# zju3dv/LoFTR

Measured on AMD Instinct MI355X. Metric: image-pairs/sec @640x480 indoor-ds, higher is better.
Workload: dtype f32; 1 GPU; batch=8 640x480 synthetic grayscale pairs per GPU, indoor_ds dual-softmax (BASELINE configs[1]), full LoFTR.forward = ResNet-FPN backbone (HIP implicit-GEMM / patch convolutions incl. the 7x7 stem) + HIP matching path; weights=seeded random init (no checkpoint on the box), conf_matrix_materialised=True, match_type=dual_softmax, global_batch=8, parallelism=dp1 (pairs sharded; RCCL all-gather of match counts)

## Files before the change

include/loftr_hip.h:

```cpp
#ifndef LOFTR_HIP_H_
#define LOFTR_HIP_H_

#include <stddef.h>
#include <stdint.h>

#ifdef __cplusplus
extern "C" {
#endif

typedef enum {
  LOFTR_OK = 0,
  LOFTR_ERR_BAD_ARG = -1,
  LOFTR_ERR_UNSUPPORTED = -2,
  LOFTR_ERR_WORKSPACE = -3,
  LOFTR_ERR_LAUNCH = -4,
  LOFTR_ERR_NO_DEVICE = -5,
  LOFTR_ERR_COMM = -6,
  LOFTR_ERR_RANGE = -7
} loftr_status;

#define LOFTR_HIP_ABI_VERSION 25

int loftr_hip_abi_version(void);
const char* loftr_hip_status_string(int status);
// ... 126 lines not shown
                                 const float* merge_b, float* out0, float* out1, void* ws,
                                 size_t ws_bytes, void* stream);

int loftr_window_head(const uint32_t* h_sp0, const uint32_t* h_sp1, int N, int H, int Wm, int Cin,
                      const void* prepared, size_t prepared_bytes, int Cout, const int64_t* b_ids,
                      const int64_t* i_ids, const int64_t* j_ids, int M, int w0c, int w1c, int stride, int W,
                      uint32_t* win0_sp, uint32_t* win1_sp, void* stream);
int loftr_fine_preprocess_window_head(const uint32_t* h_sp0, const uint32_t* h_sp1, int N, int H, int Wm, int Cin,
                                      const void* prepared, size_t prepared_bytes,
                                      const float* feat_c0, const float* feat_c1, int L, int S, int Cc,
                                      const int64_t* b_ids, const int64_t* i_ids, const int64_t* j_ids, int M,
                                      int w0c, int w1c, int stride, int W, int Cf,
                                      const float* down_w, const float* down_b, const float* merge_w,
                                      const float* merge_b, float* out0, float* out1, void* ws, size_t ws_bytes,
                                      void* stream);

int loftr_fine_match(const float* feat_f0, const float* feat_f1, int M, int WW, int C,
                     const float* mkpts1_c, const int64_t* b_ids, float scale,
                     const float* scale1, float* expec_f, float* mkpts1_f, void* stream);

size_t loftr_conv_workspace_bytes(int Cin, int Cout, int KH, int KW);
int loftr_conv_bn_act(const uint32_t* x_sp, int B, int H, int W, int Cin, const float* weight,
                      const long* weight_strides, int Cout, int KH, int KW, int stride, int pad, const float* bn_weight, const float* bn_bias,
                      const float* bn_mean, const float* bn_var, float bn_eps, int act,
                      const uint32_t* residual_sp, uint32_t* y_sp, float* y_f32, void* ws, size_t ws_bytes,
                      const float* x_inv_scale, void* stream);
int loftr_conv_prepare(const float* weight, const long* weight_strides, int Cin, int Cout, int KH, int KW,
                       const float* bn_weight, const float* bn_bias, const float* bn_mean, const float* bn_var,
                       float bn_eps, void* prepared, size_t prepared_bytes, void* stream);
#define LOFTR_CONV_SHARED_GPU 0x100
// ... 122 lines not shown
```

loftr_amd/_lib.py:

```python
import ctypes as C
import os

HERE = os.path.dirname(os.path.abspath(__file__))
LIB_PATH = os.environ.get("LOFTR_HIP_LIB") or os.path.join(HERE, "libloftr_hip.so")

_p = C.c_void_p
_i = C.c_int
_f = C.c_float
_sz = C.c_size_t
_l = C.c_long


class LayerWeights(C.Structure):
    _fields_ = [(n, _p) for n in ("q_proj", "k_proj", "v_proj", "merge", "mlp0", "mlp2",
                                  "norm1_w", "norm1_b", "norm2_w", "norm2_b")]


class CoarseParams(C.Structure):
    _fields_ = [("N", _i), ("h0c", _i), ("w0c", _i), ("h1c", _i), ("w1c", _i), ("C", _i),
                ("thr", _f), ("border_rm", _i), ("scale", _f),
                ("mask0", _p), ("mask1", _p), ("scale0", _p), ("scale1", _p)]


class MatchOut(C.Structure):
# ... 36 lines not shown
    "loftr_coarse_match_sinkhorn": (_i, [_p, _p, C.POINTER(CoarseParams), _f, _i, _i, _p, _p, C.POINTER(MatchOut),
                                         _p, _sz, _p]),
    "loftr_fine_preprocess_workspace_bytes": (_sz, [_i, _i, _i]),
    "loftr_fine_preprocess": (_i, [C.POINTER(FMap), C.POINTER(FMap), _p, _p, _i, _i, _i, _p, _p, _p, _i, _i, _i, _i,
                                   _i, _i, _p, _p, _p, _p, _p, _p, _p, _sz, _p]),
    "loftr_fine_preprocess_bwd_workspace_bytes": (_sz, [_i, _i, _i, _i]),
    "loftr_fine_preprocess_bwd": (_i, [C.POINTER(FMap), C.POINTER(FMap), _p, _p, _i, _i, _i, _p, _p, _p, _i, _i, _i, _i, _i, _i,
                                       _p, _p, _p, _p, _p, C.POINTER(FMap), C.POINTER(FMap), _p, _p, _p, _p, _p, _p, _p, _sz, _p]),
    "loftr_fine_match": (_i, [_p, _p, _i, _i, _i, _p, _p, _f, _p, _p, _p, _p]),
    "loftr_pos_encode_flatten_gather": (_i, [C.POINTER(FMap), _i, _p, _i, _p, _i, _i, _p, _i, _p]),
    "loftr_fine_preprocess_gather": (_i, [C.POINTER(FMap), _i, _p, C.POINTER(FMap), _i, _p, _p, _p, _i, _i, _i, _p, _p, _p, _i, _i, _i, _i,
                                          _i, _i, _p, _p, _p, _p, _p, _p, _p, _sz, _p]),
    "loftr_window_head": (_i, [_p, _p, _i, _i, _i, _i, _p, _sz, _i, _p, _p, _p, _i, _i, _i, _i, _i, _p, _p, _p]),
    "loftr_fine_preprocess_window_head": (_i, [_p, _p, _i, _i, _i, _i, _p, _sz, _p, _p, _i, _i, _i, _p, _p, _p, _i, _i, _i, _i,
                                               _i, _i, _p, _p, _p, _p, _p, _p, _p, _sz, _p]),
    "loftr_conv_workspace_bytes": (_sz, [_i, _i, _i, _i]),
    "loftr_conv_bn_act": (_i, [_p, _i, _i, _i, _i, _p, C.POINTER(_l), _i, _i, _i, _i, _i, _p, _p, _p, _p, _f, _i, _p, _p, _p, _p, _sz, _p, _p]),
    "loftr_stem_conv_bn_relu": (_i, [_p, C.POINTER(_l), _i, _i, _i, _p, C.POINTER(_l), _i, _p, _p, _p, _p, _f, _p, _p]),
    "loftr_upsample2x_add": (_i, [_p, _p, _p, _i, _i, _i, _i, _p]),
    "loftr_bn_train_workspace_bytes": (_sz, [_i, _i, _l]),
    "loftr_bn_train_fwd": (_i, [_p, _i, _i, _l, _i, _p, _p, _f, _p, _p, _p, _p, _p, _sz, _p]),
    "loftr_bn_train_bwd": (_i, [_p, _p, _i, _i, _l, _i, _p, _p, _p, _p, _p, _p, _p, _sz, _p]),
    "loftr_act_fwd": (_i, [_p, _p, _l, _i, _f, _p, _p]),
    "loftr_act_bwd": (_i, [_p, _p, _l, _i, _f, _p, _p]),
    "loftr_upsample2x_bilinear_fwd": (_i, [_p, _i, _i, _i, _i, _i, _p, _p]),
    "loftr_upsample2x_bilinear_bwd": (_i, [_p, _i, _i, _i, _i, _i, _p, _p]),
    "loftr_resize_linear_u8": (_i, [_p, _i, _i, _l, _p, _i, _i, _l, _p]),
    "loftr_pack_gray_u8": (_i, [_p, _l, _l, _p, _i, _i, _i, _p, _p, _p, _i, _p]),
    "loftr_epipolar_errors": (_i, [_p, _p, _p, _p, _p, _p, _l, _i, _p, _p]),
    "loftr_spvs_coarse_workspace_bytes": (_sz, [_i, _i, _i]),
# ... 79 lines not shown
```

loftr_amd/backbone.py:

```python
import os

import torch
import torch.nn as nn
import torch.nn.functional as F

from . import autograd, ops

FUSE_TOPDOWN = os.environ.get("LOFTR_FUSE_TOPDOWN", "1") != "0"


TRAIN_CONV_HIP = os.environ.get("LOFTR_TRAIN_CONV", "1") != "0"


class Conv2d(nn.Conv2d):

    def forward(self, x):
        if (TRAIN_CONV_HIP and self.training and x.is_cuda and x.dtype == torch.float32 and torch.is_grad_enabled()
                and self.in_channels <= 256 and (x.requires_grad or self.weight.requires_grad)):
            return autograd.conv2d(x, self.weight, self.stride[0], self.padding[0])
        return super().forward(x)


TRAIN_GLUE_HIP = os.environ.get("LOFTR_TRAIN_GLUE", "1") != "0"
GLUE_PARTS = set(os.environ.get("LOFTR_TRAIN_GLUE_PARTS", "bn,act,add,up").split(","))
# ... 165 lines not shown
        self.layer1_outconv2 = _fuse_head(d2, d1)
        self._init()

    def forward(self, x):
        x0 = self.relu(self.bn1(self.conv1(x)))
        x1 = self.layer1(x0)
        x2 = self.layer2(x1)
        x3 = self.layer3(x2)
        x3_out = self.layer3_outconv(x3)
        x2_out = self.layer2_outconv2(self.layer2_outconv(x2) + self._up(x3_out))
        x1_out = self.layer1_outconv2(self.layer1_outconv(x1) + self._up(x2_out))
        return [x3_out, x1_out]

    WINDOW_HEAD = "layer1_outconv2"

    def fine_head_last(self, h_sp):
        head = self.layer1_outconv2
        _, x1_f32 = ops.conv_bn_act(h_sp, head[0].out_channels, head[3], None, act=0, want_sp=False, want_f32=True)
        return self._nchw_view(x1_f32)

    @torch.no_grad()
    def forward_hip(self, x, defer_fine=False, head_input=False):
        assert defer_fine or not head_input
        a0 = self._stem_hip(x)
        a1 = self._stage_hip(self.layer1, a0)
        a2 = self._stage_hip(self.layer2, a1)
        a3 = self._stage_hip(self.layer3, a2)
        d3 = self.layer3_outconv.out_channels
        x3_sp, x3_f32 = ops.conv_bn_act(a3[0], a3[1], self.layer3_outconv, want_f32=True)

        def fine():
            t2 = self._topdown_hip(a2, self.layer2_outconv, x3_sp, d3)
            x2_out, _ = self._head_hip(self.layer2_outconv2, (t2, d3), want_f32=False, shared_gpu=defer_fine)
            d2 = self.layer2_outconv2[3].out_channels
            t1 = self._topdown_hip(a1, self.layer1_outconv, x2_out, d2)
            if head_input:
                head = self.layer1_outconv2
                return ops.conv_bn_act(t1, d2, head[0], head[1], act=2, shared_gpu=defer_fine)[0]
            _, x1_f32 = self._head_hip(self.layer1_outconv2, (t1, d2), want_f32=True, shared_gpu=defer_fine)
            return self._nchw_view(x1_f32)

        if defer_fine:
            fine.reads = (a1[0], a2[0], x3_sp)
            return [self._nchw_view(x3_f32), fine]
        return [self._nchw_view(x3_f32), fine()]


class ResNetFPN_16_4(_ResNetFPN):
    _HIP_STAGES = ("layer1", "layer2", "layer3", "layer4")
    _HIP_OUTCONVS = ("layer4_outconv", "layer3_outconv", "layer2_outconv")
# ... 64 lines not shown
```

loftr_amd/build.py:

```python
import os
import subprocess
import sys
from concurrent.futures import ThreadPoolExecutor

HERE = os.path.dirname(os.path.abspath(__file__))
CSRC = os.path.join(HERE, "csrc")
OBJ_DIR = os.path.join(CSRC, "build")
LIB_PATH = os.path.join(HERE, "libloftr_hip.so")
SOURCES = ["linear.hip", "coarse_plan.hip", "attention.hip", "transformer.hip", "coarse_match.hip", "fine.hip", "misc.hip",
           "sp_convert.hip", "conv.hip", "eval.hip", "input.hip", "comm.hip", "pose.hip", "train.hip", "train_bwd.hip", "encoder_fused.hip", "fine_fused.hip", "head_grads.hip", "encoder_bwd.hip", "fine_bwd.hip", "train_glue.hip", "bank.hip", "pose_gpu.hip", "window_head.hip", "geometry.hip", "geometry_gpu.hip"]
FLAGS = ["--offload-arch=gfx950", "-O3", "-std=c++17", "-fPIC", "-Wall", "-Wno-unused-parameter"]


def _hipcc():
    for c in (os.environ.get("HIPCC"), "/opt/rocm/bin/hipcc", "hipcc"):
        if c and (os.path.isabs(c) and os.path.exists(c) or not os.path.isabs(c)):
            return c
    raise RuntimeError("hipcc not found")


def _deps_mtime():
    paths = [os.path.join(CSRC, f) for f in os.listdir(CSRC) if f.endswith((".h", ".hip"))]
    paths.append(os.path.join(os.path.dirname(HERE), "include", "loftr_hip.h"))
    return max(os.path.getmtime(p) for p in paths)

# ... 51 lines not shown
```

loftr_amd/loftr.py:

```python
import contextlib
import math
import warnings
import weakref

import torch
import torch.nn as nn

from . import autograd, ops
from .backbone import build_backbone


class PositionEncodingSine(nn.Module):

    def __init__(self, d_model, max_shape=(256, 256), temp_bug_fix=True):
        super().__init__()
        ys = torch.arange(1, max_shape[0] + 1, dtype=torch.float32).view(1, -1, 1).expand(1, *max_shape)
        xs = torch.arange(1, max_shape[1] + 1, dtype=torch.float32).view(1, 1, -1).expand(1, *max_shape)
        idx = torch.arange(0, d_model // 2, 2).float()
        if temp_bug_fix:
            freq = torch.exp(idx * (-math.log(10000.0) / (d_model // 2)))
        else:
            freq = torch.exp(idx * (-math.log(10000.0) / d_model // 2))
        freq = freq[:, None, None]
        pe = torch.zeros((d_model, *max_shape))
# ... 214 lines not shown
        return {"b_ids": b_ids, "i_ids": i_ids, "j_ids": j_ids, "gt_mask": ~predicted, "m_bids": b_ids[predicted],
                "mkpts0_c": pts0[predicted], "mkpts1_c": pts1[predicted], "mconf": mconf[predicted]}


class FinePreprocess(nn.Module):

    def __init__(self, config):
        super().__init__()
        self.config = config
        self.cat_c_feat = config["fine_concat_coarse_feat"]
        self.W = self.config["fine_window_size"]
        d_model_c = self.config["coarse"]["d_model"]
        d_model_f = self.config["fine"]["d_model"]
        self.d_model_f = d_model_f
        self.last_head = None
        if self.cat_c_feat:
            self.down_proj = nn.Linear(d_model_c, d_model_f, bias=True)
            self.merge_feat = nn.Linear(2 * d_model_f, d_model_f, bias=True)
        for p in self.parameters():
            if p.dim() > 1:
                nn.init.kaiming_normal_(p, mode="fan_out", nonlinearity="relu")

    def forward(self, feat_f0, feat_f1, feat_c0, feat_c1, data):
        W = self.W
        stride = data["hw0_f"][0] // data["hw0_c"][0]
        data.update({"W": W})
        if data["b_ids"].shape[0] == 0:
            feat0 = torch.empty(0, self.W ** 2, self.d_model_f, device=feat_f0.device)
            feat1 = torch.empty(0, self.W ** 2, self.d_model_f, device=feat_f0.device)
            return feat0, feat1
# ... 16 lines not shown
        dense_pixels = 2 * h_sp0.shape[0] * h_sp0.shape[1] * h_sp0.shape[2]
        windows = fine_head == "windows" or ops.window_head_wins(M, dense_pixels)
        if M == 0 or not windows or not ops.window_head_supported(self.W, cin, conv.out_channels, h_sp0, h_sp1):
            self.last_head = "dense"
            if M == 0:
                return self.forward(h_sp0, h_sp1, feat_c0, feat_c1, data)
            return self.forward(dense_fn(h_sp0), dense_fn(h_sp1), feat_c0, feat_c1, data)
        self.last_head = "windows"
        W = self.W
        stride = data["hw0_f"][0] // data["hw0_c"][0]
        data.update({"W": W})
        return ops.fine_preprocess_windows(h_sp0, h_sp1, cin, conv, feat_c0, feat_c1, data["b_ids"], data["i_ids"], data["j_ids"],
                                           tuple(data["hw0_c"]), tuple(data["hw1_c"]), W, stride,
                                           down_w=self.down_proj.weight, down_b=self.down_proj.bias,
                                           merge_w=self.merge_feat.weight, merge_b=self.merge_feat.bias)

    def forward_gather(self, bank_f0, slot0, bank_f1, slot1, feat_c0, feat_c1, data):
        W = self.W
        stride = data["hw0_f"][0] // data["hw0_c"][0]
        data.update({"W": W})
        if data["b_ids"].shape[0] == 0:
            feat0 = torch.empty(0, self.W ** 2, self.d_model_f, device=bank_f0.device)
            feat1 = torch.empty(0, self.W ** 2, self.d_model_f, device=bank_f0.device)
            return feat0, feat1
        kw = {}
        if self.cat_c_feat:
            kw = dict(down_w=self.down_proj.weight, down_b=self.down_proj.bias,
                      merge_w=self.merge_feat.weight, merge_b=self.merge_feat.bias)
        return ops.fine_preprocess_gather(bank_f0, slot0, bank_f1, slot1, feat_c0, feat_c1, data["b_ids"], data["i_ids"], data["j_ids"],
                                          tuple(data["hw0_c"]), tuple(data["hw1_c"]), W, stride, **kw)
# ... 52 lines not shown
                or img0.shape[2:] != img1.shape[2:] or not hasattr(self.backbone, "WINDOW_HEAD") or not self.fine_preprocess.cat_c_feat):
            return False
        return img0.shape[0] + img1.shape[0] <= self._backbone_cap(img0)

    def _backbone_cap(self, x):
        return getattr(self, "_backbone_chunk_images", None) or max(1, (2 ** 31 - 1) // ((x.shape[2] // 2) * (x.shape[3] // 2) * 256))

    def run_backbone(self, data, head_input=False):
        data.update({"bs": data["image0"].size(0),
                     "hw0_i": data["image0"].shape[2:], "hw1_i": data["image1"].shape[2:]})
        cl = lambda img: img.contiguous(memory_format=torch.channels_last)
        use_hip = self.backbone_impl == "hip" and data["image0"].is_cuda and not self.training
        run = self.backbone.forward_hip if use_hip else self.backbone
        self._fine_join = None
        assert not head_input or (use_hip and data["hw0_i"] == data["hw1_i"])
        hkw = dict(head_input=True) if head_input else {}
        if data["hw0_i"] == data["hw1_i"]:
            x = cl(torch.cat([data["image0"], data["image1"]], dim=0))
            cap = self._backbone_cap(x)
            if use_hip and x.shape[0] > cap:
                outs = [run(x[i:i + cap]) for i in range(0, x.shape[0], cap)]
                feats_c, feats_f = torch.cat([o[0] for o in outs]), torch.cat([o[1] for o in outs])
            elif use_hip and self.overlap_fine_branch and (data["bs"] >= 8 if self.backbone_halves is None else self.backbone_halves):
                main = torch.cuda.current_stream(x.device)
                self.backbone.prepare_hip()
                if self._half_streams is None:
                    self._half_streams = [torch.cuda.Stream(device=x.device) for _ in range(2)]
                outs, fines, evs = [], [], []
                for k, st in enumerate(self._half_streams):
                    st.wait_stream(main)
                    xk = data["image0"] if k == 0 else data["image1"]
# ... 39 lines not shown
            self._fine_join = None

    def match_from_features(self, feat_c0, feat_c1, feat_f0, feat_f1, data, head_input=False):
        data.update({"hw0_c": feat_c0.shape[2:], "hw1_c": feat_c1.shape[2:]})
        if head_input:
            data.update({"hw0_f": feat_f0.shape[1:3], "hw1_f": feat_f1.shape[1:3]})
        else:
            data.update({"hw0_f": feat_f0.shape[2:], "hw1_f": feat_f1.shape[2:]})
        both = (ops.stacked_halves(feat_c0, feat_c1)
                if feat_c0.shape == feat_c1.shape and not autograd.wants_grad(feat_c0, feat_c1) else None)
        if both is not None:
            feat_c0, feat_c1 = self.pos_encoding(both).split(feat_c0.shape[0])
        else:
            feat_c0 = self.pos_encoding(feat_c0)
            feat_c1 = self.pos_encoding(feat_c1)
        if head_input:
            head = getattr(self.backbone, self.backbone.WINDOW_HEAD)
            fine_pre = lambda c0, c1: self.fine_preprocess.forward_windows(feat_f0, feat_f1, head[0].out_channels, head[3], self.backbone.fine_head_last,
                                                                           self.fine_head, c0, c1, data)
        else:
            fine_pre = lambda c0, c1: self.fine_preprocess(feat_f0, feat_f1, c0, c1, data)
        self._match_encoded(feat_c0, feat_c1, data, fine_pre)

    def _match_encoded(self, feat_c0, feat_c1, data, fine_preprocess):
        mask_c0 = mask_c1 = None
        if "mask0" in data:
            mask_c0, mask_c1 = data["mask0"].flatten(-2), data["mask1"].flatten(-2)
        feat_c0, feat_c1 = self.loftr_coarse(feat_c0, feat_c1, mask_c0, mask_c1, inplace=True, mode=self.coarse_mode,
                                             skip_padded=self.skip_padded_tiles and mask_c0 is not None)
        if not self.fine_join_late:
            self._join_fine(feat_c0.device)
# ... 17 lines not shown
            self.fine_matching(feat_f0_unfold, feat_f1_unfold, data)

    def forward(self, data):
        graph = self.training and self.full_grads and torch.is_grad_enabled()
        with torch.enable_grad() if graph else torch.no_grad():
            return self._forward(data)

    def _forward(self, data):
        dev = data["image0"].device
        if data["image1"].device != dev:
            raise ops._lib.LoftrHipError(f"image0 on {dev} but image1 on {data['image1'].device}")
        if dev.type != "cuda":
            feat_c0, feat_c1, feat_f0, feat_f1 = self.run_backbone(data)
            return self.match_from_features(feat_c0, feat_c1, feat_f0, feat_f1, data)
        with torch.cuda.device(dev):
            head_input = self._window_head_applies(data)
            feat_c0, feat_c1, feat_f0, feat_f1 = self.run_backbone(data, head_input=head_input)
            self.match_from_features(feat_c0, feat_c1, feat_f0, feat_f1, data, head_input=head_input)

    def match_pairs(self, bank0, ids0, bank1=None, ids1=None):
        from .pairs import match_pairs
        return match_pairs(self, bank0, ids0, bank1, ids1)

    def load_state_dict(self, state_dict, *args, **kwargs):
        for k in list(state_dict.keys()):
            if k.startswith("matcher."):
                state_dict[k.replace("matcher.", "", 1)] = state_dict.pop(k)
        return super().load_state_dict(state_dict, *args, **kwargs)
```

loftr_amd/ops.py:

```python
import ctypes as C
import os
import weakref
import functools

import torch

from . import _lib
from ._lib import CoarseParams, FMap, LayerWeights, MatchOut, check

_WS = {}

LAYER_FIELDS = (("q_proj", "q_proj.weight"), ("k_proj", "k_proj.weight"), ("v_proj", "v_proj.weight"),
                ("merge", "merge.weight"), ("mlp0", "mlp.0.weight"), ("mlp2", "mlp.2.weight"),
                ("norm1_w", "norm1.weight"), ("norm1_b", "norm1.bias"),
                ("norm2_w", "norm2.weight"), ("norm2_b", "norm2.bias"))


_PREPARED = weakref.WeakKeyDictionary()


def _tensors_in(obj):
    if isinstance(obj, torch.Tensor):
        yield obj
    elif isinstance(obj, (list, tuple)):
# ... 422 lines not shown
    out = torch.empty(2 * M, W * W, Cf, device=dev, dtype=torch.float32)
    out0, out1 = out[:M], out[M:]
    if M == 0:
        return out0, out1
    lib = _lib.load()
    ws = workspace(lib.loftr_fine_preprocess_workspace_bytes(M, W, Cf), dev)
    N, H, Wm, _ = h_sp0.shape
    check(lib.loftr_fine_preprocess_window_head(_ptr(h_sp0), _ptr(h_sp1), N, H, Wm, Cin, _ptr(prepared), prepared.numel(),
                                                _ptr(feat_c0), _ptr(feat_c1), feat_c0.shape[1], feat_c1.shape[1], feat_c0.shape[2],
                                                *ids, M, hw0_c[1], hw1_c[1], int(stride), int(W), Cf, _ptr(down_w), _ptr(down_b),
                                                _ptr(merge_w), _ptr(merge_b), _ptr(out0), _ptr(out1), _ptr(ws), ws.numel(),
                                                _stream()), "loftr_fine_preprocess_window_head")
    return out0, out1


def _slot_ids(ids, n_slots, name, device):
    host = ids.detach().cpu() if isinstance(ids, torch.Tensor) else torch.as_tensor(ids)
    if host.dim() != 1 or host.dtype.is_floating_point or host.dtype == torch.bool:
        raise _lib.LoftrHipError(f"{name}: expected a 1-D integer tensor of slot ids, got {tuple(host.shape)} {host.dtype}")
    if host.numel() and (int(host.min()) < 0 or int(host.max()) >= n_slots):
        raise _lib.LoftrHipError(f"{name}: slot id out of range [0, {n_slots}) (min {int(host.min())}, max {int(host.max())})")
    if isinstance(ids, torch.Tensor) and ids.is_cuda and ids.dtype == torch.int32 and ids.is_contiguous() and ids.device == device:
        return ids
    return host.to(torch.int32).to(device)


def _bank_map(bank, name):
    if not isinstance(bank, torch.Tensor) or not bank.is_cuda or bank.dtype != torch.float32 or bank.dim() != 4:
        raise _lib.LoftrHipError(f"{name}: expected a 4-D float32 GPU tensor [n_slots, C, H, W]")
    if bank.shape[0] == 0:
# ... 456 lines not shown
```

Before: 408.7 image-pairs/s.

## Compute both fine-head 3x3 convs only on matched windows instead of dense map

Moves the first 3x3 conv+BN+ReLU of layer1_outconv2 out of the dense backbone. It is now computed only over 7x7 neighbourhoods around the matched coarse cells, followed by the second conv on the 5x5 windows. A new MFMA kernel file stages patches and weights through LDS with async global-to-LDS loads. This is meant to skip dense full-resolution conv work when the total window area is small relative to the map. It falls back to the dense path when the fill ratio exceeds a threshold, and it adds a new code path that has to be kept equivalent to the dense one.

New measurement: 434.0 image-pairs/s (median of 6 runs). +6.2%, better.

```diff
diff --git a/include/loftr_hip.h b/include/loftr_hip.h
--- a/include/loftr_hip.h
+++ b/include/loftr_hip.h
@@ -164,6 +164,23 @@
                                       const float* down_w, const float* down_b, const float* merge_w,
                                       const float* merge_b, float* out0, float* out1, void* ws, size_t ws_bytes,
                                       void* stream);
+
+int loftr_window_head_first(const uint32_t* t_sp0, const uint32_t* t_sp1, int N, int H, int Wm, int Cin,
+                            const void* prepared, size_t prepared_bytes, int Cout, const int64_t* b_ids,
+                            const int64_t* i_ids, const int64_t* j_ids, int M, int w0c, int w1c, int stride, int W,
+                            uint32_t* nb_sp, void* stream);
+int loftr_window_head_last(const uint32_t* nb_sp, int H, int Wm, int Cin, const void* prepared, size_t prepared_bytes,
+                           int Cout, const int64_t* b_ids, const int64_t* i_ids, const int64_t* j_ids, int M, int w0c,
+                           int w1c, int stride, int W, uint32_t* win0_sp, uint32_t* win1_sp, void* stream);
+int loftr_fine_preprocess_window_head2(const uint32_t* t_sp0, const uint32_t* t_sp1, int N, int H, int Wm, int Cin,
+                                       const void* prepared0, size_t prepared0_bytes, int Cmid,
+                                       const void* prepared1, size_t prepared1_bytes,
+                                       const float* feat_c0, const float* feat_c1, int L, int S, int Cc,
+                                       const int64_t* b_ids, const int64_t* i_ids, const int64_t* j_ids, int M,
+                                       int w0c, int w1c, int stride, int W, int Cf,
+                                       const float* down_w, const float* down_b, const float* merge_w,
+                                       const float* merge_b, float* out0, float* out1, void* ws, size_t ws_bytes,
+                                       uint32_t* nb_sp, void* stream);
 
 int loftr_fine_match(const float* feat_f0, const float* feat_f1, int M, int WW, int C,
                      const float* mkpts1_c, const int64_t* b_ids, float scale,
diff --git a/loftr_amd/_lib.py b/loftr_amd/_lib.py
--- a/loftr_amd/_lib.py
+++ b/loftr_amd/_lib.py
@@ -74,6 +74,10 @@
     "loftr_window_head": (_i, [_p, _p, _i, _i, _i, _i, _p, _sz, _i, _p, _p, _p, _i, _i, _i, _i, _i, _p, _p, _p]),
     "loftr_fine_preprocess_window_head": (_i, [_p, _p, _i, _i, _i, _i, _p, _sz, _p, _p, _i, _i, _i, _p, _p, _p, _i, _i, _i, _i,
                                                _i, _i, _p, _p, _p, _p, _p, _p, _p, _sz, _p]),
+    "loftr_window_head_first": (_i, [_p, _p, _i, _i, _i, _i, _p, _sz, _i, _p, _p, _p, _i, _i, _i, _i, _i, _p, _p]),
+    "loftr_window_head_last": (_i, [_p, _i, _i, _i, _p, _sz, _i, _p, _p, _p, _i, _i, _i, _i, _i, _p, _p, _p]),
+    "loftr_fine_preprocess_window_head2": (_i, [_p, _p, _i, _i, _i, _i, _p, _sz, _i, _p, _sz, _p, _p, _i, _i, _i, _p, _p, _p, _i, _i, _i,
+                                                _i, _i, _i, _p, _p, _p, _p, _p, _p, _p, _sz, _p, _p]),
     "loftr_conv_workspace_bytes": (_sz, [_i, _i, _i, _i]),
     "loftr_conv_bn_act": (_i, [_p, _i, _i, _i, _i, _p, C.POINTER(_l), _i, _i, _i, _i, _i, _p, _p, _p, _p, _f, _i, _p, _p, _p, _p, _sz, _p, _p]),
     "loftr_stem_conv_bn_relu": (_i, [_p, C.POINTER(_l), _i, _i, _i, _p, C.POINTER(_l), _i, _p, _p, _p, _p, _f, _p, _p]),
diff --git a/loftr_amd/backbone.py b/loftr_amd/backbone.py
--- a/loftr_amd/backbone.py
+++ b/loftr_amd/backbone.py
@@ -203,6 +203,10 @@
 
     WINDOW_HEAD = "layer1_outconv2"
 
+    def fine_head_first(self, t_sp):
+        head = self.layer1_outconv2
+        return ops.conv_bn_act(t_sp, head[0].in_channels, head[0], head[1], act=2)[0]
+
     def fine_head_last(self, h_sp):
         head = self.layer1_outconv2
         _, x1_f32 = ops.conv_bn_act(h_sp, head[0].out_channels, head[3], None, act=0, want_sp=False, want_f32=True)
@@ -223,6 +227,8 @@
             x2_out, _ = self._head_hip(self.layer2_outconv2, (t2, d3), want_f32=False, shared_gpu=defer_fine)
             d2 = self.layer2_outconv2[3].out_channels
             t1 = self._topdown_hip(a1, self.layer1_outconv, x2_out, d2)
+            if head_input == "t1":
+                return t1
             if head_input:
                 head = self.layer1_outconv2
                 return ops.conv_bn_act(t1, d2, head[0], head[1], act=2, shared_gpu=defer_fine)[0]
diff --git a/loftr_amd/build.py b/loftr_amd/build.py
--- a/loftr_amd/build.py
+++ b/loftr_amd/build.py
@@ -8,7 +8,7 @@
 OBJ_DIR = os.path.join(CSRC, "build")
 LIB_PATH = os.path.join(HERE, "libloftr_hip.so")
 SOURCES = ["linear.hip", "coarse_plan.hip", "attention.hip", "transformer.hip", "coarse_match.hip", "fine.hip", "misc.hip",
-           "sp_convert.hip", "conv.hip", "eval.hip", "input.hip", "comm.hip", "pose.hip", "train.hip", "train_bwd.hip", "encoder_fused.hip", "fine_fused.hip", "head_grads.hip", "encoder_bwd.hip", "fine_bwd.hip", "train_glue.hip", "bank.hip", "pose_gpu.hip", "window_head.hip", "geometry.hip", "geometry_gpu.hip"]
+           "sp_convert.hip", "conv.hip", "eval.hip", "input.hip", "comm.hip", "pose.hip", "train.hip", "train_bwd.hip", "encoder_fused.hip", "fine_fused.hip", "head_grads.hip", "encoder_bwd.hip", "fine_bwd.hip", "train_glue.hip", "bank.hip", "pose_gpu.hip", "window_head.hip", "window_head_first.hip", "geometry.hip", "geometry_gpu.hip"]
 FLAGS = ["--offload-arch=gfx950", "-O3", "-std=c++17", "-fPIC", "-Wall", "-Wno-unused-parameter"]
 
 
diff --git a/loftr_amd/csrc/window_head_first.hip b/loftr_amd/csrc/window_head_first.hip
--- /dev/null
+++ b/loftr_amd/csrc/window_head_first.hip
@@ -0,0 +1,403 @@
+#include "conv_prepared.h"
+#include "fine.h"
+
+namespace whf {
+
+constexpr int NWIN = 5;
+constexpr int NB = 4, LA = NB - 1;
+
+template <int OUT_, int NT_, int WM_, int WN_, int RW_, bool PACKED_>
+struct Cfg {
+  static constexpr int OUT = OUT_, PS = OUT_ + 2, OO = OUT_ * OUT_, PP = PS * PS;
+  static constexpr int NT = NT_, WM = WM_, WN = WN_, RW = RW_, WAVES = WM_ * WN_, NJ = (NT_ + WN_ - 1) / WN_;
+  static constexpr bool PACKED = PACKED_;
+  static constexpr int ROWS = WM * RW * 32;
+  static constexpr int PROWS = NWIN * PP, PSLOTS = (PROWS + 15) / 16, PQ = (PSLOTS + WAVES - 1) / WAVES;
+  static constexpr int PHALF_BYTES = PSLOTS * 1024;
+  static constexpr int BSLOTS = NT * 32 / 16, BQ = (BSLOTS + WAVES - 1) / WAVES, BSTAGE_BYTES = BSLOTS * 1024;
+  static constexpr int SCR_OFF = 2 * PHALF_BYTES + NB * BSTAGE_BYTES;
+  static constexpr int TAB_OFF = SCR_OFF + 1024;
+  static constexpr int LDS_BYTES = TAB_OFF + ROWS * 8;
+  static constexpr int WG_PER_CU = WAVES == 4 ? 2 : 1;
+  static_assert(NWIN * OO <= ROWS, "the windows' output pixels fit the tile rows");
+  static_assert(LDS_BYTES * WG_PER_CU <= 160 * 1024, "LDS");
+  static_assert(WN == 1 || NT - (WN - 1) * NJ >= NJ - 1, "the last column split owns NJ or NJ - 1 tiles");
+};
+using First = Cfg<7, 7, 4, 2, 2, false>;
+using Last = Cfg<5, 4, 4, 1, 1, true>;
+
+struct Args {
+  const sp_t* x0; const sp_t* x1;
+  int H, W, Cp, Cin;
+  const sp_t* w; int K;
+  const float* bias; const float* wscale;
+  const sp_t* zeros;
+  const int64_t* b_ids; const int64_t* i_ids; const int64_t* j_ids;
+  int M, w0c, w1c, stride;
+  int Cout;
+  int act;
+  sp_t* out0; sp_t* out1;
+};
+
+struct WinPos { int b, y0, x0, side; };
+template <int OUT>
+__device__ __forceinline__ WinPos window_pos(const Args& p, int w) {
+  const int side = w >= p.M ? 1 : 0, m = w - side * p.M;
+  const long cell = side ? p.j_ids[m] : p.i_ids[m];
+  const int wc = side ? p.w1c : p.w0c;
+  WinPos o;
+  o.b = (int)p.b_ids[m];
+  o.y0 = (int)(cell / wc) * p.stride - OUT / 2;
+  o.x0 = (int)(cell % wc) * p.stride - OUT / 2;
+  o.side = side;
+  return o;
+}
+
+template <typename CF>
+__global__ __launch_bounds__(CF::WAVES * 64, CF::WG_PER_CU) void window_nbhd_kernel(Args p) {
+  constexpr int OUT = CF::OUT, PS = CF::PS, OO = CF::OO, PP = CF::PP, NT = CF::NT, RW = CF::RW, NJ = CF::NJ;
+  constexpr int WAVES = CF::WAVES, WM = CF::WM, ROWS = CF::ROWS, PQ = CF::PQ, BQ = CF::BQ;
+  typedef __attribute__((address_space(3))) void* lds_ptr_t;
+  typedef const __attribute__((address_space(1))) void* gbl_ptr_t;
+  __shared__ __attribute__((aligned(16))) char lds[CF::LDS_BYTES];
+  char* const patch_base = lds;
+  char* const bring_base = lds + 2 * CF::PHALF_BYTES;
+  char* const scratch = lds + CF::SCR_OFF;
+  int* const row_off = reinterpret_cast<int*>(lds + CF::TAB_OFF);
+  int* const row_flag = row_off + ROWS;
+
+  const int tile = blockIdx.x, nwin = 2 * p.M;
+  const int tid = threadIdx.x, lane = tid & 63, wave = tid >> 6;
+  const int g = lane >> 5, tx = lane & 31;
+  const int wr = wave % WM, wn = wave / WM;
+  const int jc0 = wn * NJ;
+  const int nj = min(NJ, NT - jc0);
+  const int drow = lane >> 2, dpos = lane & 3;
+
+  if (tid < ROWS) {
+    const int wl = tid / OO, px = tid - wl * OO, w = tile * NWIN + wl;
+    int off = -1, flag = 0;
+    if (wl < NWIN && w < nwin) {
+      const WinPos wp = window_pos<OUT>(p, w);
+      const int y = wp.y0 + px / OUT, x = wp.x0 + px % OUT;
+      const bool in = (unsigned)y < (unsigned)p.H && (unsigned)x < (unsigned)p.W;
+      off = ((w - wp.side * p.M) * OO + px) * (NT * 32);
+      flag = wp.side | (in ? 2 : 0);
+    }
+    row_off[tid] = off;
+    row_flag[tid] = flag;
+  }
+
+  int poff[PQ];
+  unsigned pside = 0;
+#pragma unroll
+  for (int q = 0; q < PQ; ++q) {
+    const int s_ = q * WAVES + wave, r = s_ * 16 + drow;
+    const int wl = r / PP, rem = r - wl * PP, py = rem / PS, px = rem - py * PS;
+    const int w = tile * NWIN + wl;
+    const bool live = s_ < CF::PSLOTS && r < CF::PROWS && w < nwin;
+    const WinPos wp = window_pos<OUT>(p, live ? w : 0);
+    const int c = dpos ^ ((r >> 2) & 3);
+    const int coff = ((c & 1) + ((c >> 1) << 2)) << 2;
+    if (CF::PACKED) {
+      poff[q] = live ? ((w - wp.side * p.M) * PP + rem) * p.Cp + coff : -1;
+    } else {
+      const int gy = wp.y0 - 1 + py, gx = wp.x0 - 1 + px;
+      const bool in = live && (unsigned)gy < (unsigned)p.H && (unsigned)gx < (unsigned)p.W;
+      poff[q] = in ? ((wp.b * p.H + gy) * p.W + gx) * p.Cp + coff : -1;
+    }
+    pside |= (unsigned)wp.side << q;
+  }
+  int boff[BQ];
+#pragma unroll
+  for (int q = 0; q < BQ; ++q) {
+    const int r = (q * WAVES + wave) * 16 + drow;
+    const int c = dpos ^ ((r >> 2) & 3);
+    boff[q] = min(r, p.Cout - 1) * p.K + (((c & 1) + ((c >> 1) << 2)) << 2);
+  }
+  const int gpt = p.Cp >> 5;
+  const int nhalf = 2 * gpt - (p.Cin <= (gpt - 1) * 32 + 16 ? 1 : 0), ns = nhalf * 9;
+
+#define WHF_ISSUE_PATCH(q_)                                                                                 \
+  {                                                                                                         \
+    const sp_t* xa__ = p.x0;                                                                                \
+    const sp_t* xb__ = p.x1;                                                                                \
+    asm volatile("" : "+s"(xa__), "+s"(xb__));                                                              \
+    const int ko__ = ((q_) >> 1) * 32 + ((q_) & 1) * 8;                                                     \
+    char* dst__ = patch_base + ((q_) & 1) * CF::PHALF_BYTES;                                                \
+    _Pragma("unroll") for (int q = 0; q < PQ; ++q) {                                                        \
+      const sp_t* g__ = poff[q] >= 0 ? (((pside >> q) & 1u) ? xb__ : xa__) + (poff[q] + ko__) : p.zeros;    \
+      char* d__ = (q * WAVES + wave < CF::PSLOTS) ? dst__ + (q * WAVES + wave) * 1024 : scratch;            \
+      __builtin_amdgcn_global_load_lds((gbl_ptr_t)g__, (lds_ptr_t)d__, 16, 0, 0);                           \
+    }                                                                                                       \
+  }
+#define WHF_ISSUE_B(q_, i_, stage_)                                                                         \
+  {                                                                                                         \
+    const sp_t* wb__ = p.w;                                                                                 \
+    asm volatile("" : "+s"(wb__));                                                                          \
+    const int kx__ = (i_) / 3, ky__ = (i_) - kx__ * 3;                                                      \
+    const int ko__ = (ky__ * 3 + kx__) * p.Cp + ((q_) >> 1) * 32 + ((q_) & 1) * 8;                          \
+    char* dst__ = bring_base + (stage_) * CF::BSTAGE_BYTES;                                                 \
+    _Pragma("unroll") for (int q = 0; q < BQ; ++q) {                                                        \
+      char* d__ = (q * WAVES + wave < CF::BSLOTS) ? dst__ + (q * WAVES + wave) * 1024 : scratch;            \
+      __builtin_amdgcn_global_load_lds((gbl_ptr_t)(wb__ + (boff[q] + ko__)), (lds_ptr_t)d__, 16, 0, 0);     \
+    }                                                                                                       \
+  }
+
+  f32x16 acc[RW][NJ];
+#pragma unroll
+  for (int i = 0; i < RW; ++i)
+#pragma unroll
+    for (int j = 0; j < NJ; ++j)
+#pragma unroll
+      for (int r = 0; r < 16; ++r) acc[i][j][r] = 0.f;
+
+  int bbase[NJ];
+#pragma unroll
+  for (int j = 0; j < NJ; ++j) {
+    const int br = min(jc0 + j, NT - 1) * 32 + tx;
+    bbase[j] = br * 64 + ((g ^ ((br >> 2) & 3)) << 4);
+  }
+  int arow[RW];
+#pragma unroll
+  for (int i = 0; i < RW; ++i) {
+    const int r = (wr * RW + i) * 32 + tx, wl = r / OO, px = r - wl * OO;
+    arow[i] = wl < NWIN ? wl * PP + (px / OUT) * PS + px % OUT : 0;
+  }
+#define WHF_LOAD_A(h_, l_, sP_, i_, toff_)                                                                  \
+  {                                                                                                         \
+    const int pr__ = arow[i_] + (toff_);                                                                    \
+    const int ab__ = pr__ * 64 + ((g ^ ((pr__ >> 2) & 3)) << 4);                                            \
+    h_ = *reinterpret_cast<const h16x8*>((sP_) + ab__);                                                     \
+    l_ = *reinterpret_cast<const h16x8*>((sP_) + (ab__ ^ 32));                                              \
+  }
+#define WHF_LOAD_B(h_, l_, off_)        \
+  {                                                                                                         \
+    h_ = *reinterpret_cast<const h16x8*>(bring_base + (off_));                                              \
+    l_ = *reinterpret_cast<const h16x8*>(bring_base + ((off_) ^ 32));                                       \
+  }
+
+  WHF_ISSUE_PATCH(0);
+#pragma unroll
+  for (int s = 0; s < LA; ++s) WHF_ISSUE_B(0, s, s);
+  int q3 = 0, i3 = LA;
+  int stage = 0;
+  bool patch_m1 = false, patch_m2 = false;
+  h16x8 ah[RW], al[RW], bh0, bl0;
+  LOFTR_WAITCNT_VM((LA - 1) * BQ);
+  __builtin_amdgcn_s_barrier();
+#pragma unroll
+  for (int i = 0; i < RW; ++i) WHF_LOAD_A(ah[i], al[i], patch_base, i, 0);
+  WHF_LOAD_B(bh0, bl0, bbase[0]);
+
+  __builtin_amdgcn_s_setprio(1);
+  int s = 0;
+  for (int hq = 0; hq < nhalf; ++hq) {
+    const char* sP = patch_base + (hq & 1) * CF::PHALF_BYTES;
+    const char* sPn = patch_base + ((hq + 1) & 1) * CF::PHALF_BYTES;
+#pragma unroll
+    for (int i = 0; i < 9; ++i) {
+      {
+        const bool w2 = s + 2 < ns;
+        const bool pp = patch_m1 || patch_m2;
+        if (w2 && pp) LOFTR_WAITCNT_VM(BQ + PQ);
+        else if (pp) LOFTR_WAITCNT_VM(PQ);
+        else if (w2) LOFTR_WAITCNT_VM(BQ);
+        else LOFTR_WAITCNT_VM(0);
+      }
+      __builtin_amdgcn_s_barrier();
+      if (s + LA < ns) WHF_ISSUE_B(q3, i3, stage + LA >= NB ? stage + LA - NB : stage + LA);
+      if (++i3 == 9) { i3 = 0; ++q3; }
+      patch_m2 = patch_m1;
+      patch_m1 = false;
+      if (i == 0 && hq + 1 < nhalf) { WHF_ISSUE_PATCH(hq + 1); patch_m1 = true; }
+      const int nstage = stage + 1 == NB ? 0 : stage + 1;
+      const int sB = stage * CF::BSTAGE_BYTES, sBn = nstage * CF::BSTAGE_BYTES;
+      h16x8 nah[RW], nal[RW];
+#pragma unroll
+      for (int ii = 0; ii < RW; ++ii) {
+        if (i < 8) { WHF_LOAD_A(nah[ii], nal[ii], sP, ii, ((i + 1) % 3) * PS + (i + 1) / 3); }
+        else { WHF_LOAD_A(nah[ii], nal[ii], sPn, ii, 0); }
+      }
+      h16x8 ch = bh0, cl = bl0;
+#pragma unroll
+      for (int j = 0; j < NJ; ++j) {
+        if (CF::WN > 1 && j >= nj) continue;
+        h16x8 nh, nl;
+        const bool more = j + 1 < NJ && (CF::WN == 1 || j + 1 < nj);
+        const int nb = more ? sB + bbase[j + 1 < NJ ? j + 1 : 0] : sBn + bbase[0];
+        WHF_LOAD_B(nh, nl, nb);
+#pragma unroll
+        for (int ii = 0; ii < RW; ++ii) acc[ii][j] = __builtin_amdgcn_mfma_f32_32x32x16_f16(al[ii], ch, acc[ii][j], 0, 0, 0);
+#pragma unroll
+        for (int ii = 0; ii < RW; ++ii) acc[ii][j] = __builtin_amdgcn_mfma_f32_32x32x16_f16(ah[ii], cl, acc[ii][j], 0, 0, 0);
+#pragma unroll
+        for (int ii = 0; ii < RW; ++ii) acc[ii][j] = __builtin_amdgcn_mfma_f32_32x32x16_f16(ah[ii], ch, acc[ii][j], 0, 0, 0);
+        ch = nh; cl = nl;
+      }
+      bh0 = ch; bl0 = cl;
+#pragma unroll
+      for (int ii = 0; ii < RW; ++ii) { ah[ii] = nah[ii]; al[ii] = nal[ii]; }
+      stage = nstage;
+      ++s;
+    }
+  }
+#undef WHF_LOAD_B
+#undef WHF_LOAD_A
+#undef WHF_ISSUE_B
+#undef WHF_ISSUE_PATCH
+  __builtin_amdgcn_s_setprio(0);
+
+  const bool odd = lane & 1;
+  const float slope = p.act == 1 ? 0.f : p.act == 2 ? 0.01f : 1.f;
+#pragma unroll
+  for (int i = 0; i < RW; ++i) {
+    int roff[16], rflag[16];
+#pragma unroll
+    for (int r = 0; r < 16; ++r) {
+      const int row = (wr * RW + i) * 32 + (r & 3) + 8 * (r >> 2) + 4 * g;
+      roff[r] = row_off[row];
+      rflag[r] = row_flag[row];
+    }
+#pragma unroll
+    for (int j = 0; j < NJ; ++j) {
+      if (CF::WN > 1 && j >= nj) continue;
+      const int col = (jc0 + j) * 32 + tx, colc = min(col, p.Cout - 1);
+      const bool creal = col < p.Cout;
+      const float bia = p.bias ? p.bias[colc] : 0.f;
+      const float wsc = p.wscale[colc];
+      f32x16 v;
+#pragma unroll
+      for (int r = 0; r < 16; ++r) {
+        const float xv = fmaf(acc[i][j][r], wsc, bia);
+        v[r] = creal ? fmaxf(xv, slope * xv) : 0.f;
+      }
+      uint32_t w16[16];
+      sp_words16(v, odd, w16);
+      const int lane_sp = (jc0 + j) * 32 + (odd ? 16 : 0) + (tx >> 1);
+#pragma unroll
+      for (int r = 0; r < 16; ++r) {
+        if (roff[r] >= 0) {
+          sp_t* o = (rflag[r] & 1) ? p.out1 : p.out0;
+          o[(unsigned)(roff[r] + lane_sp)] = (rflag[r] & 2) ? w16[r] : 0u;
+        }
+      }
+    }
+  }
+}
+
+struct HeadWindows2 { Args first, last; sp_t* nb; };
+
+template <typename CF>
+int launch(Args a, sp_t* out0, sp_t* out1, hipStream_t st) {
+  a.out0 = out0; a.out1 = out1;
+  hipLaunchKernelGGL((window_nbhd_kernel<CF>), dim3(ceil_div(2 * a.M, NWIN)), dim3(CF::WAVES * 64), 0, st, a);
+  LOFTR_CHECK_LAUNCH();
+  return LOFTR_OK;
+}
+
+int launch_first(const HeadWindows2& h, hipStream_t st) {
+  return launch<First>(h.first, h.nb, h.nb + (size_t)h.first.M * First::OO * (First::NT * 32), st);
+}
+
+int launch_head_windows2(const void* ctx, sp_t* win0, sp_t* win1, hipStream_t st) {
+  const HeadWindows2& h = *(const HeadWindows2*)ctx;
+  const int rc = launch_first(h, st);
+  if (rc != LOFTR_OK) return rc;
+  return launch<Last>(h.last, win0, win1, st);
+}
+
+int ids_args(const int64_t* b_ids, const int64_t* i_ids, const int64_t* j_ids, int M, int w0c, int w1c, int stride, int W, Args& a) {
+  LOFTR_CHECK_ARG(b_ids && i_ids && j_ids && M > 0 && w0c > 0 && w1c > 0 && stride > 0);
+  if (W != Last::OUT) return LOFTR_ERR_UNSUPPORTED;
+  if ((long)2 * M * First::OO * (First::NT * 32) >= (1L << 31)) return LOFTR_ERR_UNSUPPORTED;
+  a.b_ids = b_ids; a.i_ids = i_ids; a.j_ids = j_ids; a.M = M; a.w0c = w0c; a.w1c = w1c; a.stride = stride;
+  a.out0 = nullptr; a.out1 = nullptr;
+  return LOFTR_OK;
+}
+
+int first_args(const uint32_t* t_sp0, const uint32_t* t_sp1, int N, int H, int Wm, int Cin, const void* prepared, size_t prepared_bytes,
+               int Cout, const int64_t* b_ids, const int64_t* i_ids, const int64_t* j_ids, int M, int w0c, int w1c, int stride, int W,
+               Args& a) {
+  LOFTR_CHECK_ARG(t_sp0 && t_sp1 && prepared && N > 0 && H > 0 && Wm > 0 && Cin > 0 && Cout > 0);
+  const int rc = ids_args(b_ids, i_ids, j_ids, M, w0c, w1c, stride, W, a);
+  if (rc != LOFTR_OK) return rc;
+  if (Cin != 196 || Cout != 196) return LOFTR_ERR_UNSUPPORTED;
+  const int Cp = ceil32(Cin);
+  if ((long)N * H * Wm * Cp >= (1L << 31)) return LOFTR_ERR_UNSUPPORTED;
+  ConvPrepared pr;
+  if (!conv_prepared_layout(const_cast<void*>(prepared), prepared_bytes, Cin, Cout, 3, 3, pr)) return LOFTR_ERR_WORKSPACE;
+  a.x0 = t_sp0; a.x1 = t_sp1; a.H = H; a.W = Wm; a.Cp = Cp; a.Cin = Cin;
+  a.w = pr.wsp; a.K = 9 * Cp; a.bias = pr.bias; a.wscale = pr.wscale; a.zeros = pr.zeros;
+  a.Cout = Cout; a.act = 2;
+  return LOFTR_OK;
+}
+
+int last_args(const uint32_t* nb_sp, int H, int Wm, int Cin, const void* prepared, size_t prepared_bytes, int Cout,
+              const int64_t* b_ids, const int64_t* i_ids, const int64_t* j_ids, int M, int w0c, int w1c, int stride, int W, Args& a) {
+  LOFTR_CHECK_ARG(nb_sp && prepared && H > 0 && Wm > 0 && Cin > 0 && Cout > 0);
+  const int rc = ids_args(b_ids, i_ids, j_ids, M, w0c, w1c, stride, W, a);
+  if (rc != LOFTR_OK) return rc;
+  if (Cin != 196 || Cout != 128) return LOFTR_ERR_UNSUPPORTED;
+  const int Cp = ceil32(Cin);
+  ConvPrepared pr;
+  if (!conv_prepared_layout(const_cast<void*>(prepared), prepared_bytes, Cin, Cout, 3, 3, pr)) return LOFTR_ERR_WORKSPACE;
+  a.x0 = nb_sp; a.x1 = nb_sp + (size_t)M * Last::PP * Cp; a.H = H; a.W = Wm; a.Cp = Cp; a.Cin = Cin;
+  a.w = pr.wsp; a.K = 9 * Cp; a.bias = pr.bias; a.wscale = pr.wscale; a.zeros = pr.zeros;
+  a.Cout = Cout; a.act = 0;
+  return LOFTR_OK;
+}
+
+static_assert(Last::PP == First::OO && First::NT * 32 == 224, "the last kernel's patch rows are the first kernel's output rows");
+
+}
+
+extern "C" int loftr_window_head_first(const uint32_t* t_sp0, const uint32_t* t_sp1, int N, int H, int Wm, int Cin,
+                                       const void* prepared, size_t prepared_bytes, int Cout, const int64_t* b_ids,
+                                       const int64_t* i_ids, const int64_t* j_ids, int M, int w0c, int w1c, int stride, int W,
+                                       uint32_t* nb_sp, void* stream) {
+  LOFTR_CHECK_ARG(M >= 0);
+  if (M == 0) return LOFTR_OK;
+  LOFTR_CHECK_ARG(nb_sp);
+  whf::HeadWindows2 h;
+  const int rc = whf::first_args(t_sp0, t_sp1, N, H, Wm, Cin, prepared, prepared_bytes, Cout, b_ids, i_ids, j_ids, M, w0c, w1c, stride,
+                                 W, h.first);
+  if (rc != LOFTR_OK) return rc;
+  h.nb = nb_sp;
+  return whf::launch_first(h, (hipStream_t)stream);
+}
+
+extern "C" int loftr_window_head_last(const uint32_t* nb_sp, int H, int Wm, int Cin, const void* prepared, size_t prepared_bytes,
+                                      int Cout, const int64_t* b_ids, const int64_t* i_ids, const int64_t* j_ids, int M, int w0c,
+                                      int w1c, int stride, int W, uint32_t* win0_sp, uint32_t* win1_sp, void* stream) {
+  LOFTR_CHECK_ARG(M >= 0);
+  if (M == 0) return LOFTR_OK;
+  LOFTR_CHECK_ARG(win0_sp && win1_sp);
+  whf::Args a;
+  const int rc = whf::last_args(nb_sp, H, Wm, Cin, prepared, prepared_bytes, Cout, b_ids, i_ids, j_ids, M, w0c, w1c, stride, W, a);
+  if (rc != LOFTR_OK) return rc;
+  return whf::launch<whf::Last>(a, win0_sp, win1_sp, (hipStream_t)stream);
+}
+
+extern "C" int loftr_fine_preprocess_window_head2(const uint32_t* t_sp0, const uint32_t* t_sp1, int N, int H, int Wm, int Cin,
+                                                  const void* prepared0, size_t prepared0_bytes, int Cmid,
+                                                  const void* prepared1, size_t prepared1_bytes,
+                                                  const float* feat_c0, const float* feat_c1, int L, int S, int Cc,
+                                                  const int64_t* b_ids, const int64_t* i_ids, const int64_t* j_ids, int M,
+                                                  int w0c, int w1c, int stride, int W, int Cf,
+                                                  const float* down_w, const float* down_b, const float* merge_w,
+                                                  const float* merge_b, float* out0, float* out1, void* ws, size_t ws_bytes,
+                                                  uint32_t* nb_sp, void* stream) {
+  LOFTR_CHECK_ARG(M >= 0);
+  if (M == 0) return LOFTR_OK;
+  LOFTR_CHECK_ARG(out0 && out1 && Cf > 0 && nb_sp && prepared0 && prepared1);
+  whf::HeadWindows2 h;
+  int rc = whf::first_args(t_sp0, t_sp1, N, H, Wm, Cin, prepared0, prepared0_bytes, Cmid, b_ids, i_ids, j_ids, M, w0c, w1c, stride, W,
+                           h.first);
+  if (rc != LOFTR_OK) return rc;
+  rc = whf::last_args(nb_sp, H, Wm, Cmid, prepared1, prepared1_bytes, Cf, b_ids, i_ids, j_ids, M, w0c, w1c, stride, W, h.last);
+  if (rc != LOFTR_OK) return rc;
+  h.nb = nb_sp;
+  return fine_preprocess_run(WindowGather{whf::launch_head_windows2, &h}, feat_c0, feat_c1, L, S, Cc, b_ids, i_ids, j_ids, M, W, Cf,
+                             down_w, down_b, merge_w, merge_b, out0, out1, ws, ws_bytes, (hipStream_t)stream);
+}
diff --git a/loftr_amd/loftr.py b/loftr_amd/loftr.py
--- a/loftr_amd/loftr.py
+++ b/loftr_amd/loftr.py
@@ -252,6 +252,7 @@
         d_model_f = self.config["fine"]["d_model"]
         self.d_model_f = d_model_f
         self.last_head = None
+        self.last_head_first = None
         if self.cat_c_feat:
             self.down_proj = nn.Linear(d_model_c, d_model_f, bias=True)
             self.merge_feat = nn.Linear(2 * d_model_f, d_model_f, bias=True)
@@ -298,6 +299,30 @@
                                            tuple(data["hw0_c"]), tuple(data["hw1_c"]), W, stride,
                                            down_w=self.down_proj.weight, down_b=self.down_proj.bias,
                                            merge_w=self.merge_feat.weight, merge_b=self.merge_feat.bias)
+
+    def forward_windows2(self, t_sp0, t_sp1, cin, head, first_fn, dense_fn, fine_head, feat_c0, feat_c1, data):
+        M = data["b_ids"].shape[0]
+        dense_pixels = 2 * t_sp0.shape[0] * t_sp0.shape[1] * t_sp0.shape[2]
+        both = (M > 0 and (fine_head == "windows" or ops.window_head_first_wins(M, dense_pixels))
+                and ops.window_head_first_supported(self.W, cin, head[0], head[3], t_sp0, t_sp1, M))
+        if not both:
+            self.last_head_first = "dense"
+            if M == 0:
+                return self.forward_windows(t_sp0, t_sp1, head[0].out_channels, head[3], dense_fn, fine_head, feat_c0, feat_c1, data)
+            stacked = ops.stacked_halves(t_sp0, t_sp1)
+            if stacked is not None:
+                h_sp0, h_sp1 = first_fn(stacked).split(t_sp0.shape[0])
+            else:
+                h_sp0, h_sp1 = first_fn(t_sp0), first_fn(t_sp1)
+            return self.forward_windows(h_sp0, h_sp1, head[0].out_channels, head[3], dense_fn, fine_head, feat_c0, feat_c1, data)
+        self.last_head = self.last_head_first = "windows"
+        W = self.W
+        stride = data["hw0_f"][0] // data["hw0_c"][0]
+        data.update({"W": W})
+        return ops.fine_preprocess_windows2(t_sp0, t_sp1, cin, head[0], head[1], head[3], feat_c0, feat_c1, data["b_ids"], data["i_ids"],
+                                            data["j_ids"], tuple(data["hw0_c"]), tuple(data["hw1_c"]), W, stride,
+                                            down_w=self.down_proj.weight, down_b=self.down_proj.bias,
+                                            merge_w=self.merge_feat.weight, merge_b=self.merge_feat.bias)
 
     def forward_gather(self, bank_f0, slot0, bank_f1, slot1, feat_c0, feat_c1, data):
         W = self.W
@@ -380,7 +405,7 @@
         run = self.backbone.forward_hip if use_hip else self.backbone
         self._fine_join = None
         assert not head_input or (use_hip and data["hw0_i"] == data["hw1_i"])
-        hkw = dict(head_input=True) if head_input else {}
+        hkw = dict(head_input=head_input) if head_input else {}
         if data["hw0_i"] == data["hw1_i"]:
             x = cl(torch.cat([data["image0"], data["image1"]], dim=0))
             cap = self._backbone_cap(x)
@@ -450,7 +475,11 @@
         else:
             feat_c0 = self.pos_encoding(feat_c0)
             feat_c1 = self.pos_encoding(feat_c1)
-        if head_input:
+        if head_input == "t1":
+            head = getattr(self.backbone, self.backbone.WINDOW_HEAD)
+            fine_pre = lambda c0, c1: self.fine_preprocess.forward_windows2(feat_f0, feat_f1, head[0].in_channels, head, self.backbone.fine_head_first,
+                                                                            self.backbone.fine_head_last, self.fine_head, c0, c1, data)
+        elif head_input:
             head = getattr(self.backbone, self.backbone.WINDOW_HEAD)
             fine_pre = lambda c0, c1: self.fine_preprocess.forward_windows(feat_f0, feat_f1, head[0].out_channels, head[3], self.backbone.fine_head_last,
                                                                            self.fine_head, c0, c1, data)
@@ -498,7 +527,7 @@
             feat_c0, feat_c1, feat_f0, feat_f1 = self.run_backbone(data)
             return self.match_from_features(feat_c0, feat_c1, feat_f0, feat_f1, data)
         with torch.cuda.device(dev):
-            head_input = self._window_head_applies(data)
+            head_input = "t1" if self._window_head_applies(data) else False
             feat_c0, feat_c1, feat_f0, feat_f1 = self.run_backbone(data, head_input=head_input)
             self.match_from_features(feat_c0, feat_c1, feat_f0, feat_f1, data, head_input=head_input)
 
diff --git a/loftr_amd/ops.py b/loftr_amd/ops.py
--- a/loftr_amd/ops.py
+++ b/loftr_amd/ops.py
@@ -460,6 +460,88 @@
     return out0, out1
 
 
+WINDOW_HEAD_FIRST_MAX_FILL = 0.85
+
+
+def window_head_first_wins(M, dense_pixels):
+    return window_head_wins(M, dense_pixels) and 2 * M * 49 <= WINDOW_HEAD_FIRST_MAX_FILL * dense_pixels
+
+
+def window_head_first_supported(W, Cin, conv0, conv1, t_sp0, t_sp1, M):
+    return (window_head_supported(W, Cin, conv1.out_channels, t_sp0, t_sp1) and Cin == 196 and conv0.out_channels == 196
+            and conv1.in_channels == 196 and 2 * M * 49 * 224 < 2 ** 31)
+
+
+def _window_head_first_common(t_sp0, t_sp1, Cin, conv, bn, b_ids, i_ids, j_ids):
+    for t, n in ((t_sp0, "t_sp0"), (t_sp1, "t_sp1")):
+        if not t.is_cuda or t.dtype != torch.int32 or not t.is_contiguous() or t.dim() != 4:
+            raise _lib.LoftrHipError(f"{n}: expected a contiguous int32 (SP) GPU tensor [N, H, W, Cp]")
+    if t_sp0.shape != t_sp1.shape or t_sp0.shape[3] != ceil32(Cin):
+        raise _lib.LoftrHipError(f"window head: SP maps {tuple(t_sp0.shape)} / {tuple(t_sp1.shape)} for {Cin} channels")
+    Cout, Cin_w, KH, KW = conv.weight.shape
+    if (Cin_w, KH, KW) != (Cin, 3, 3) or conv.stride[0] != 1 or conv.padding[0] != 1:
+        raise _lib.LoftrHipError("window head: a 3x3 / stride-1 / pad-1 convolution expected")
+    ids = [_ptr(_need(t, n, torch.int64)) for t, n in ((b_ids, "b_ids"), (i_ids, "i_ids"), (j_ids, "j_ids"))]
+    return Cout, _prepared_conv(conv, bn), ids
+
+
+@_on_device
+def window_head_first(t_sp0, t_sp1, Cin, conv, bn, b_ids, i_ids, j_ids, hw0_c, hw1_c, W, stride):
+    Cout, prepared, ids = _window_head_first_common(t_sp0, t_sp1, Cin, conv, bn, b_ids, i_ids, j_ids)
+    M = b_ids.shape[0]
+    nb = torch.empty(2 * M, 49, ceil32(Cout), dtype=torch.int32, device=t_sp0.device)
+    if M:
+        N, H, Wm, _ = t_sp0.shape
+        check(_lib.load().loftr_window_head_first(_ptr(t_sp0), _ptr(t_sp1), N, H, Wm, Cin, _ptr(prepared), prepared.numel(), Cout, *ids,
+                                                  M, hw0_c[1], hw1_c[1], int(stride), int(W), _ptr(nb), _stream()),
+              "loftr_window_head_first")
+    return nb
+
+
+@_on_device
+def window_head_last(nb, hw_f, Cin, conv, b_ids, i_ids, j_ids, hw0_c, hw1_c, W, stride):
+    M = b_ids.shape[0]
+    if not nb.is_cuda or nb.dtype != torch.int32 or not nb.is_contiguous() or tuple(nb.shape) != (2 * M, 49, ceil32(Cin)):
+        raise _lib.LoftrHipError(f"nb: expected a contiguous int32 (SP) GPU tensor [{2 * M}, 49, {ceil32(Cin)}]")
+    Cout = conv.weight.shape[0]
+    prepared = _prepared_conv(conv, None)
+    ids = [_ptr(_need(t, n, torch.int64)) for t, n in ((b_ids, "b_ids"), (i_ids, "i_ids"), (j_ids, "j_ids"))]
+    win = torch.empty(2, M, W * W, ceil32(Cout), dtype=torch.int32, device=nb.device)
+    if M:
+        check(_lib.load().loftr_window_head_last(_ptr(nb), int(hw_f[0]), int(hw_f[1]), Cin, _ptr(prepared), prepared.numel(), Cout, *ids,
+                                                 M, hw0_c[1], hw1_c[1], int(stride), int(W), _ptr(win[0]), _ptr(win[1]), _stream()),
+              "loftr_window_head_last")
+    return win[0], win[1]
+
+
+@_on_device
+def fine_preprocess_windows2(t_sp0, t_sp1, Cin, conv0, bn0, conv1, feat_c0, feat_c1, b_ids, i_ids, j_ids, hw0_c, hw1_c, W, stride,
+                             down_w, down_b, merge_w, merge_b):
+    Cmid, prepared0, ids = _window_head_first_common(t_sp0, t_sp1, Cin, conv0, bn0, b_ids, i_ids, j_ids)
+    Cf = conv1.weight.shape[0]
+    if tuple(conv1.weight.shape[1:]) != (Cmid, 3, 3) or conv1.stride[0] != 1 or conv1.padding[0] != 1:
+        raise _lib.LoftrHipError("window head: a 3x3 / stride-1 / pad-1 second convolution expected")
+    prepared1 = _prepared_conv(conv1, None)
+    _need(feat_c0, "feat_c0"); _need(feat_c1, "feat_c1")
+    M = b_ids.shape[0]
+    dev = t_sp0.device
+    out = torch.empty(2 * M, W * W, Cf, device=dev, dtype=torch.float32)
+    out0, out1 = out[:M], out[M:]
+    if M == 0:
+        return out0, out1
+    lib = _lib.load()
+    ws = workspace(lib.loftr_fine_preprocess_workspace_bytes(M, W, Cf), dev)
+    nb = torch.empty(2 * M, 49, ceil32(Cmid), dtype=torch.int32, device=dev)
+    N, H, Wm, _ = t_sp0.shape
+    check(lib.loftr_fine_preprocess_window_head2(_ptr(t_sp0), _ptr(t_sp1), N, H, Wm, Cin, _ptr(prepared0), prepared0.numel(), Cmid,
+                                                 _ptr(prepared1), prepared1.numel(),
+                                                 _ptr(feat_c0), _ptr(feat_c1), feat_c0.shape[1], feat_c1.shape[1], feat_c0.shape[2],
+                                                 *ids, M, hw0_c[1], hw1_c[1], int(stride), int(W), Cf, _ptr(down_w), _ptr(down_b),
+                                                 _ptr(merge_w), _ptr(merge_b), _ptr(out0), _ptr(out1), _ptr(ws), ws.numel(),
+                                                 _ptr(nb), _stream()), "loftr_fine_preprocess_window_head2")
+    return out0, out1
+
+
 def _slot_ids(ids, n_slots, name, device):
     host = ids.detach().cpu() if isinstance(ids, torch.Tensor) else torch.as_tensor(ids)
     if host.dim() != 1 or host.dtype.is_floating_point or host.dtype == torch.bool:
```
